# JiuTongBro/vqnerf_release

Measured on AMD Instinct MI355X. Metric: rays/sec (render) 800x800, 64+64 samples/ray, NeuS SDF 8x256 + colour 4x256, higher is better.
Workload: dtype f32; 1 GPU; BASELINE configs[1], nerf/hotdog-shaped NeuS render: one whole 800x800 pin-hole view per rank per step (camera at distance 4, fov 0.6911), n_samples=64, n_importance=64, up_sample_steps=4, sdf 8x256; parallelism=views x1 (no data-path collective)

## Files before the change

vqnerf_release_amd/csrc/mlp_prims.h:

```cpp
#pragma once
#include "common.h"

namespace eng {

enum Act : int { ACT_NONE = 0, ACT_RELU = 1, ACT_SOFTPLUS100 = 2, ACT_SIGMOID = 3 };

__device__ __forceinline__ float fast_exp(float x) { return __builtin_amdgcn_exp2f(x * 1.4426950408889634f); }
__device__ __forceinline__ float fast_log(float x) { return __builtin_amdgcn_logf(x) * 0.6931471805599453f; }
__device__ __forceinline__ float fast_rcp(float x) { return __builtin_amdgcn_rcpf(x); }

template <int ACT>
__device__ __forceinline__ float act_fwd(float x) {
  if (ACT == ACT_RELU) return fmaxf(x, 0.f);
  if (ACT == ACT_SOFTPLUS100) {
    const float t = 100.f * x;
    return t > 20.f ? x : 0.01f * fast_log(1.f + fast_exp(t));
  }
  if (ACT == ACT_SIGMOID) return fast_rcp(1.f + fast_exp(-x));
  return x;
}

template <int ACT>
__device__ __forceinline__ float act_bwd_from_out(float h) {
  if (ACT == ACT_RELU) return h > 0.f ? 1.f : 0.f;
// ... 391 lines not shown
  const f32x4* b = bpack + ot * 8;
  const bool hi = lane >= 32;
#pragma unroll
  for (int rq = 0; rq < 4; ++rq) {
    const f32x4 v0 = b[rq], v1 = b[4 + rq];
    acc[4 * rq + 0] = hi ? v1[0] : v0[0]; acc[4 * rq + 1] = hi ? v1[1] : v0[1];
    acc[4 * rq + 2] = hi ? v1[2] : v0[2]; acc[4 * rq + 3] = hi ? v1[3] : v0[3];
  }
}

__device__ __forceinline__ void init_zero(f32x16& acc) {
#pragma unroll
  for (int i = 0; i < 16; ++i) acc[i] = 0.f;
}

__device__ __forceinline__ void init_rows(const f32x4* __restrict__ rows , int lane, f32x16& acc) {
#pragma unroll
  for (int rq = 0; rq < 4; ++rq) {
    f32x4 v = rows[rq * 64 + lane];
    acc[4 * rq + 0] = v[0]; acc[4 * rq + 1] = v[1]; acc[4 * rq + 2] = v[2]; acc[4 * rq + 3] = v[3];
  }
}

__device__ __forceinline__ float posenc_feat(int f, float x0, float x1, float x2) {
  if (f < 3) return f == 0 ? x0 : (f == 1 ? x1 : x2);
  const int g = f - 3, k = g / 6, m = g - 6 * k, c = m >= 3 ? m - 3 : m;
  const float xc = c == 0 ? x0 : (c == 1 ? x1 : x2);
  const float arg = xc * (float)(1 << k);
  return m < 3 ? sinf(arg) : cosf(arg);
}
__device__ __forceinline__ float posenc_jac(int f, float x0, float x1, float x2, int* comp) {
  if (f < 3) { *comp = f; return 1.f; }
  const int g = f - 3, k = g / 6, m = g - 6 * k, c = m >= 3 ? m - 3 : m;
  const float xc = c == 0 ? x0 : (c == 1 ? x1 : x2);
  const float fr = (float)(1 << k), arg = xc * fr;
  *comp = c;
  return m < 3 ? fr * cosf(arg) : -fr * sinf(arg);
}

__device__ __forceinline__ int row_feat(int r, int h, int j) { return 32 * (r >> 2) + 2 * (4 * (r & 3) + j) + h; }
__device__ __forceinline__ float lds_feat(const f32x4* __restrict__ lds, const int row0, const int f, const int pp) {
  const int t = f >> 5, fi = f & 31, hh = fi & 1, rr = fi >> 1;
  return reinterpret_cast<const float*>(lds)[(((row0 + t * 4 + (rr >> 2)) * 64) + pp + 32 * hh) * 4 + (rr & 3)];
}

template <int NOUT, int NW = 4>
// ... 36 lines not shown
```

vqnerf_release_amd/csrc/neus_launch.h:

```cpp
#pragma once
#include "neus_phases.h"
#include "launch.h"
#include <stdio.h>


static int neus_sdf_args(const char* fn, const int32_t* sdf_desc, const float* wbuf_sdf, const float* rays_o, const float* rays_d,
                         const float* z, const float* pts, const int64_t P, const int S, const float* out_sdf,
                         int (*check_desc)(const SdfDesc&), const char* desc_msg, SdfDesc* sd) {
  VQN_CHECK_ARG_IN(fn, sdf_desc && wbuf_sdf && out_sdf, "sdf_desc, wbuf_sdf, out_sdf must be non-null");
  VQN_CHECK_ARG_IN(fn, P >= 0, "P >= 0");
  if (P == 0) return VQN_OK;
  VQN_CHECK_ARG_IN(fn, pts != nullptr || (rays_o && rays_d && z && S > 0), "either pts or (rays_o, rays_d, z, S) required");
  memcpy(sd, sdf_desc, sizeof(SdfDesc));
  VQN_CHECK_SHAPE_IN(fn, check_desc(*sd) == 0, desc_msg);
  return VQN_OK;
}

static int neus_fine_args(const char* fn, const int32_t* sdf_desc, const float* wbuf_sdf, const int32_t* col_desc, const float* wbuf_col,
                          const float* rays_o, const float* rays_d, const float* z, const float* pts, const float* dirs, const int64_t P,
                          const int S, const void* scratch, const float* out_sdf, const float* out_grad, const float* out_rgb,
                          int (*check_desc)(const SdfDesc&), const char* desc_msg, bool (*extras_rows_ok)(const ColDesc&),
                          SdfDesc* sd, ColDesc* cd) {
  VQN_CHECK_ARG_IN(fn, sdf_desc && wbuf_sdf && col_desc && wbuf_col, "descriptors and weight packs must be non-null");
  VQN_CHECK_ARG_IN(fn, out_sdf && out_grad && scratch, "out_sdf, out_grad and scratch must be non-null");
// ... 8 lines not shown
    VQN_CHECK_ARG_IN(fn, out_rgb != nullptr, "out_rgb must be non-null when a colour net is given");
    VQN_CHECK_SHAPE_IN(fn, sd->layers[sd->n_lin - 1].n_out_tiles >= 1, "SDF network has no feature outputs (d_out == 1)");
    VQN_CHECK_SHAPE_IN(fn, cd->n_lin >= 2 && cd->n_lin <= VQN_MAX_COL_LAYERS && cd->d_out == 3, "colour net: 2..8 layers, d_out == 3");
    VQN_CHECK_SHAPE_IN(fn, cd->extra_feats >= 3 && cd->extra_feats <= 64 && extras_rows_ok(*cd), "colour net extras");
    for (int l = 0; l < cd->n_lin - 1; ++l)
      VQN_CHECK_SHAPE_IN(fn, cd->layers[l].n_out_tiles >= 1 && cd->layers[l].n_out_tiles <= sd->max_tiles, "colour layer wider than max_tiles");
  }
  return VQN_OK;
}

static eng::TrainOut neus_train_out(float* const* tensors, const int nL, const int nC, const int e_tiles, const int outf_tiles, const int extr_tiles) {
  eng::TrainOut to;
  memset(&to, 0, sizeof(to));
  to.E = tensors[0]; to.OUTF = tensors[1]; to.EXTR = tensors[2];
  for (int l = 1; l <= nL; ++l) to.U[l] = tensors[3 + (l - 1)];
  for (int l = 0; l < nL; ++l) to.GH[l] = tensors[3 + nL + l];
  for (int l = 1; l <= nC; ++l) to.C[l] = tensors[3 + 2 * nL + (l - 1)];
  to.e_tiles = e_tiles; to.outf_tiles = outf_tiles; to.extr_tiles = extr_tiles;
  return to;
}

static int64_t neus_stash_bytes(const SdfDesc& sd) { return (int64_t)(sd.n_lin - 1) * 4 * sd.max_tiles * 1024; }

static long pair_grid(const long n_tiles, const int images, const int64_t per_img, const int64_t scratch_bytes) {
  return vqn_grid_in_scratch(vqn_grid((n_tiles + images - 1) / images, images == 1 ? 2 : 1), images * per_img, scratch_bytes);
}

constexpr int TB_MAX_L = 12;

struct TrainBwdDesc {
  int nL, nC, skip, emb_rows, emb_feats, e_tiles, max_tiles, feat_tiles;
  int outf_tiles, squeeze, offBtop, offWrow, offCBfeat, offCBnrm;
  float scale, inv_scale;
  int ts[TB_MAX_L];
  int tc[TB_MAX_L];
  int offT[TB_MAX_L];
  int offB[TB_MAX_L];
  int offCB[TB_MAX_L];
};
constexpr int TB_DESC_INTS = 16 + 5 * TB_MAX_L;
static_assert(sizeof(TrainBwdDesc) == TB_DESC_INTS * 4, "descriptor layout");

struct TrainBwdPtrs {
  const float* X; const float* G_RGB; const float* RGB; const float* G_N; const float* G_SDF;
  const float* U[TB_MAX_L];
  const float* GH[TB_MAX_L];
  const float* C[TB_MAX_L];
  float* DC[TB_MAX_L];
// ... 29 lines not shown
  VQN_CHECK_ARG_IN(fn, desc && w0 && w1 && pts && g_rgb && scratch && saved && outs, "null pointer");
  VQN_CHECK_ARG_IN(fn, P >= 1, "P >= 1");
  VQN_CHECK_SHAPE_IN(fn, train_bwd_load_desc(desc, engine_rules, bd) == 0, desc_msg);
  const int nL = bd->nL, nC = bd->nC;
  VQN_CHECK_ARG_IN(fn, n_saved == 2 * nL + nC, "saved: [U_1..U_nL, GH_0..GH_{nL-1}, C_1..C_nC]");
  VQN_CHECK_ARG_IN(fn, n_outs == (nC + 1) + 2 + 2 * nL, "outs: [DC_0..DC_nC, GOUTF, ED, UD_1..UD_nL, AB_0..AB_{nL-1}]");
  VQN_CHECK_ARG_IN(fn, (rgb != nullptr) == (bd->squeeze != 0), "rgb: the forward's colours when the colour net ends in a sigmoid, else NULL");
  for (int i = 0; i < n_saved; ++i) VQN_CHECK_ARG_IN(fn, saved[i] != nullptr, "null saved tensor");
  for (int i = 0; i < n_outs; ++i) VQN_CHECK_ARG_IN(fn, outs[i] != nullptr, "null output tensor");
  const int64_t per_img = train_bwd_stash_bytes(*bd);
  char scratch_msg[96];
  snprintf(scratch_msg, sizeof(scratch_msg), "scratch too small (see %s_scratch_bytes)", fn);
  VQN_CHECK_ARG_IN(fn, scratch_bytes >= 2 * per_img, scratch_msg);
  memset(tp, 0, sizeof(*tp));
  tp->X = pts; tp->G_RGB = g_rgb; tp->RGB = rgb; tp->G_N = g_n; tp->G_SDF = g_sdf;
  for (int l = 1; l <= nL; ++l) tp->U[l] = saved[l - 1];
  for (int l = 0; l < nL; ++l) tp->GH[l] = saved[nL + l];
  for (int l = 1; l <= nC; ++l) tp->C[l] = saved[2 * nL + l - 1];
  for (int l = 0; l <= nC; ++l) tp->DC[l] = outs[l];
  tp->GOUTF = outs[nC + 1];
  tp->ED = outs[nC + 2];
  for (int l = 1; l <= nL; ++l) tp->UD[l] = outs[nC + 3 + l - 1];
  for (int l = 0; l < nL; ++l) tp->AB[l] = outs[nC + 3 + nL + l];
  *grid = pair_grid((P + 31) / 32, 2, per_img, scratch_bytes);
  return VQN_OK;
}
```

vqnerf_release_amd/csrc/neus_mlp.hip:

```cpp
#include "neus_launch.h"
#include <stdlib.h>

using namespace eng;

#ifdef VQN_STAMPS
__device__ unsigned long long g_stamps[8];
#define VQN_STAMP_DECL unsigned long long st_[6] = {0, 0, 0, 0, 0, 0}; unsigned long long st_prev = __builtin_amdgcn_s_memtime(); const unsigned long long st_begin = st_prev;
#define VQN_STAMP(i) { const unsigned long long st_now = __builtin_amdgcn_s_memtime(); st_[i] += st_now - st_prev; st_prev = st_now; }
#define VQN_STAMP_FLUSH if (threadIdx.x == 0) { st_[5] = __builtin_amdgcn_s_memtime() - st_begin; for (int i_ = 0; i_ < 6; ++i_) atomicAdd(&g_stamps[i_], st_[i_]); atomicAdd(&g_stamps[6], 1ull); }
extern "C" int vqn_debug_read_stamps(unsigned long long* out, int reset) {
  if (hipMemcpyFromSymbol(out, HIP_SYMBOL(g_stamps), sizeof(unsigned long long) * 8) != hipSuccess) return -3;
  if (reset) { unsigned long long z[8] = {0, 0, 0, 0, 0, 0, 0, 0}; if (hipMemcpyToSymbol(HIP_SYMBOL(g_stamps), z, sizeof(z)) != hipSuccess) return -3; }
  return 0;
}
#else
#define VQN_STAMP_DECL
#define VQN_STAMP(i)
#define VQN_STAMP_FLUSH
#endif

#ifdef VQN_STAMPS
__device__ unsigned long long g_stamps2[16];
#define FS_DECL unsigned long long fs_[16] = {0, 0, 0, 0, 0, 0, 0, 0, 0, 0, 0, 0, 0, 0, 0, 0}; unsigned long long fs_prev = __builtin_amdgcn_s_memtime(); const unsigned long long fs_begin = fs_prev;
#define FS(i) { const unsigned long long fs_now = __builtin_amdgcn_s_memtime(); fs_[i] += fs_now - fs_prev; fs_prev = fs_now; }
// ... 610 lines not shown
      if (wave < L.n_out_tiles) {
#pragma unroll
        for (int im = 0; im < NIMG; ++im) {
#pragma unroll
          for (int rq = 0; rq < 4; ++rq) lds[(size_t)im * IS + (X0 + wave * 4 + rq) * 64 + lane] = acc_quad(acc[im], rq);
        }
      }
      __syncthreads();
    }
    const int hid_rows = 4 * sd.layers[n_lin - 2].n_out_tiles;

    for (int u = wave; u < 4 * NIMG; u += 8)
      rowdot<1>(lds + (size_t)(u >> 2) * IS, X0, hid_rows, wsdf + sd.last_w_off, sm->part[u >> 2], u & 3, lane);
    __syncthreads();
    if (tid < 32 * NIMG) {
      const int im = tid >> 5, t = tid & 31;
      const long pt = ((NIMG * grp + im) << 5) + t;
      if (pt < P) out_sdf[pt] = sdf_raw(sm->part[im], t, sd.last_b_off, sd.last_bias, wsdf) / sd.scale;
    }
    __syncthreads();
  }
}

int check_sdf_desc(const SdfDesc& d) {
  if (d.n_lin < 2 || d.n_lin > VQN_MAX_SDF_LAYERS) return 1;
  if (d.max_tiles < 1 || d.max_tiles > 16) return 2;
  if (d.emb_feats < 3 || d.emb_feats > 64 || d.emb_rows < 1 || d.emb_rows > 8) return 3;
  if (d.skip >= d.n_lin - 1 || d.skip == 0) return 4;
  for (int l = 0; l < d.n_lin; ++l)
    if (d.layers[l].n_out_tiles < 0 || d.layers[l].n_out_tiles > d.max_tiles) return 5;
  if (!(d.scale > 0.f)) return 6;
  return 0;
}

template <int NIMG>
size_t lds_bytes(int MT) { return (size_t)NIMG * (E_ROWS + 8 * MT) * 1024 + sizeof(Smalls<NIMG>); }

bool use_two_images(int MT) {
  static const bool forced32 = getenv("VQN_NEUS_TILE32") != nullptr;
  return !forced32 && MT >= 5 && lds_bytes<2>(MT) <= 160 * 1024;
}

template <int NIMG>
size_t lds_bytes_sdf(const SdfDesc& sd) { return (size_t)NIMG * (sd.emb_rows + 4 * sd.max_tiles) * 1024 + sizeof(SmallsSdf<NIMG>); }

constexpr int SDF_IMAGES_DEFAULT = 4;
int sdf_images(const SdfDesc& sd) {
  static const int cap = [] {
    const char* e = getenv("VQN_NEUS_SDF_IMAGES");
    const int v = e != nullptr ? atoi(e) : SDF_IMAGES_DEFAULT;
    return v >= 2 && v <= 4 ? v : SDF_IMAGES_DEFAULT;
  }();
  if (!use_two_images(sd.max_tiles)) return 1;
  if (sd.max_tiles <= 8) {
    if (cap >= 4 && lds_bytes_sdf<4>(sd) <= 160 * 1024) return 4;
    if (cap >= 3 && lds_bytes_sdf<3>(sd) <= 160 * 1024) return 3;
  }
  return 2;
}

template <int NIMG>
int launch_sdf_images(const char* fn, const SdfDesc& sd, const f32x4* ws, const float* rays_o, const float* rays_d, const float* z,
                      const float* pts, const int64_t P, const int S, float* out_sdf, void* stream) {
  return vqn_launch(fn, neus_pointsN_kernel<NIMG>, pair_grid((P + 31) / 32, NIMG, 0, 0), 512, lds_bytes_sdf<NIMG>(sd), stream, sd, ws,
                    rays_o, rays_d, z, pts, (long)P, S, out_sdf);
}

bool extras_rows_ok(const ColDesc& cd) { return cd.extra_rows >= 1 && cd.extra_rows <= 8; }

}

extern "C" int vqn_neus_sdf_points(const int32_t* sdf_desc, const float* wbuf_sdf, const float* rays_o,
                                   const float* rays_d, const float* z, const float* pts, int64_t P, int S,
                                   float* out_sdf, void* stream) {
  SdfDesc sd;
  const int rc = neus_sdf_args(__func__, sdf_desc, wbuf_sdf, rays_o, rays_d, z, pts, P, S, out_sdf, check_sdf_desc,
                               "invalid SDF network descriptor", &sd);
  if (rc != VQN_OK || P == 0) return rc;
  ColDesc cd;
  memset(&cd, 0, sizeof(cd));
  const long n_tiles = (P + 31) / 32;
  const f32x4* ws = reinterpret_cast<const f32x4*>(wbuf_sdf);
  const int images = sdf_images(sd);
  if (images == 4) return launch_sdf_images<4>(__func__, sd, ws, rays_o, rays_d, z, pts, P, S, out_sdf, stream);
  if (images == 3) return launch_sdf_images<3>(__func__, sd, ws, rays_o, rays_d, z, pts, P, S, out_sdf, stream);
  if (images == 2)
    return vqn_launch(__func__, neus_points2_kernel<false>, pair_grid(n_tiles, 2, 0, 0), 512, lds_bytes<2>(sd.max_tiles), stream, sd, cd, ws,
                      nullptr, rays_o, rays_d, z, pts, nullptr, (long)P, S, nullptr, out_sdf, nullptr, nullptr, TrainOut{});
  const size_t lds = lds_bytes<1>(sd.max_tiles);
  VQN_CHECK_SHAPE(lds <= 160 * 1024, "network too wide for LDS");
  return vqn_launch(__func__, neus_points_kernel<false>, pair_grid(n_tiles, 1, 0, 0), 256, lds, stream, sd, cd, ws, nullptr, rays_o, rays_d,
                    z, pts, nullptr, (long)P, S, nullptr, out_sdf, nullptr, nullptr);
}

extern "C" int vqn_neus_train_fwd(const int32_t* sdf_desc, const float* wbuf_sdf, const int32_t* col_desc, const float* wbuf_col,
                                  const float* pts, const float* dirs, int64_t P, void* scratch, int64_t scratch_bytes,
                                  float* const* tensors, int n_tensors, int e_tiles, int outf_tiles, int extr_tiles, float* out_sdf,
                                  float* out_n, float* out_rgb, void* stream) {
  VQN_CHECK_ARG(sdf_desc && wbuf_sdf && col_desc && wbuf_col && pts && dirs && scratch && tensors && out_sdf && out_n && out_rgb, "null pointer");
  VQN_CHECK_ARG(P >= 1, "P >= 1");
  SdfDesc sd;
  ColDesc cd;
  memcpy(&sd, sdf_desc, sizeof(SdfDesc));
  memcpy(&cd, col_desc, sizeof(ColDesc));
  VQN_CHECK_SHAPE(check_sdf_desc(sd) == 0, "invalid SDF network descriptor");
  VQN_CHECK_SHAPE(cd.n_lin >= 2 && cd.n_lin <= VQN_MAX_COL_LAYERS && cd.d_out == 3 && sd.layers[sd.n_lin - 1].n_out_tiles >= 1, "colour net");
  VQN_CHECK_SHAPE(use_two_images(sd.max_tiles), "the training forward kernel is the two-image form only");
  const int nL = sd.n_lin - 1, nC = cd.n_lin - 1;
  VQN_CHECK_ARG(n_tensors == 3 + 2 * nL + nC, "tensors: [E, OUTF, EXTR, U_1..U_nL, GH_0..GH_{nL-1}, C_1..C_nC]");
  VQN_CHECK_SHAPE(e_tiles * 4 >= sd.emb_rows && e_tiles <= 2 && extr_tiles * 4 >= cd.extra_rows && extr_tiles <= 2 &&
                  outf_tiles >= sd.layers[sd.n_lin - 1].n_out_tiles, "tile counts");
  for (int i = 0; i < n_tensors; ++i) VQN_CHECK_ARG(tensors[i] != nullptr, "null tensor pointer");
  const long grid = pair_grid((P + 31) / 32, 2, neus_stash_bytes(sd), scratch_bytes);
  VQN_CHECK_ARG(grid >= 1, "scratch too small (see vqn_neus_fine_scratch_bytes)");
  return vqn_launch(__func__, neus_points2_kernel<true, true>, grid, 512, lds_bytes<2>(sd.max_tiles), stream, sd, cd,
                    reinterpret_cast<const f32x4*>(wbuf_sdf), reinterpret_cast<const f32x4*>(wbuf_col), nullptr, nullptr, nullptr, pts, dirs,
                    (long)P, 1, reinterpret_cast<f32x4*>(scratch), out_sdf, out_n, out_rgb,
                    neus_train_out(tensors, nL, nC, e_tiles, outf_tiles, extr_tiles));
}

extern "C" int64_t vqn_neus_fine_scratch_bytes(const int32_t* sdf_desc) {
  if (!sdf_desc) return -1;
  SdfDesc sd;
  memcpy(&sd, sdf_desc, sizeof(SdfDesc));
  const int emb_rows = sd.emb_rows;
  if (emb_rows >= 1 && emb_rows <= 12) sd.emb_rows = 1;
  if (check_sdf_desc(sd) != 0) return -2;
#ifdef VQN_DIAG_STASH_ROT
  return (int64_t)VQN_DIAG_STASH_ROT * vqn_num_cus() * 2 * neus_stash_bytes(sd);
#else
  return (int64_t)vqn_num_cus() * 2 * neus_stash_bytes(sd);
#endif
}

extern "C" int vqn_neus_fine_points(const int32_t* sdf_desc, const float* wbuf_sdf, const int32_t* col_desc,
                                    const float* wbuf_col, const float* rays_o, const float* rays_d, const float* z,
                                    const float* pts, const float* dirs, int64_t P, int S, void* scratch,
                                    int64_t scratch_bytes, float* out_sdf, float* out_grad, float* out_rgb,
                                    void* stream) {
  SdfDesc sd;
  ColDesc cd;
  const int rc = neus_fine_args(__func__, sdf_desc, wbuf_sdf, col_desc, wbuf_col, rays_o, rays_d, z, pts, dirs, P, S, scratch, out_sdf,
                                out_grad, out_rgb, check_sdf_desc, "invalid SDF network descriptor", extras_rows_ok, &sd, &cd);
  if (rc != VQN_OK || P == 0) return rc;
  if (cd.n_lin != 0)
    VQN_CHECK_ARG((cd.reserved1 > 0 && cd.reserved2 > cd.reserved1 && cd.reserved3 > cd.reserved2) ||
                  (cd.reserved1 == 0 && cd.reserved2 == 0 && cd.reserved3 == 0), "col_desc: fold offsets (reserved1..3) inconsistent");
  const long n_tiles = (P + 31) / 32;
  const int64_t per_img = neus_stash_bytes(sd);
  const f32x4* ws = reinterpret_cast<const f32x4*>(wbuf_sdf);
  const f32x4* wc = reinterpret_cast<const f32x4*>(wbuf_col);
  if (use_two_images(sd.max_tiles)) {
    const bool fold = cd.n_lin != 0 && cd.reserved1 > 0;
#ifdef VQN_DIAG_STASH_ROT
    const long grid = pair_grid(n_tiles, 2, 0, 0);
    VQN_CHECK_ARG((int64_t)VQN_DIAG_STASH_ROT * grid * 2 * per_img <= scratch_bytes, "diag build: scratch must hold ROT regions per workgroup");
#else
    const long grid = pair_grid(n_tiles, 2, per_img, scratch_bytes);
#endif
    VQN_CHECK_ARG(grid >= 1, "scratch too small (see vqn_neus_fine_scratch_bytes)");
    return vqn_launch(__func__, fold ? neus_points2_kernel<true, false, true> : neus_points2_kernel<true>, grid, 512, lds_bytes<2>(sd.max_tiles),
                      stream, sd, cd, ws, wc, rays_o, rays_d, z, pts, dirs, (long)P, S, reinterpret_cast<f32x4*>(scratch), out_sdf, out_grad,
                      out_rgb, TrainOut{});
  }
  const size_t lds = lds_bytes<1>(sd.max_tiles);
  VQN_CHECK_SHAPE(lds <= 160 * 1024, "network too wide for LDS");
  const long grid = pair_grid(n_tiles, 1, per_img, scratch_bytes);
  VQN_CHECK_ARG(grid >= 1, "scratch too small (see vqn_neus_fine_scratch_bytes)");
  return vqn_launch(__func__, neus_points_kernel<true>, grid, 256, lds, stream, sd, cd, ws, wc, rays_o, rays_d, z, pts, dirs, (long)P, S,
                    reinterpret_cast<f32x4*>(scratch), out_sdf, out_grad, out_rgb);
}
```

vqnerf_release_amd/csrc/neus_mlp_f16s.hip:

```cpp
#include "mlp_prims_f16s.h"
#include "neus_launch.h"
#include <stdlib.h>

using namespace eng;

#define st_stream(p, ...) (*(p) = (__VA_ARGS__))
#define ld_stream(p) (*(p))

#ifdef VQN_STAMPS
__device__ unsigned long long g_stamps16[16];
#define FS_DECL unsigned long long st_[16] = {0, 0, 0, 0, 0, 0, 0, 0, 0, 0, 0, 0, 0, 0, 0, 0}; unsigned long long st_prev = __builtin_amdgcn_s_memtime(); const unsigned long long st_begin = st_prev;
#define FS(i) { const unsigned long long st_now = __builtin_amdgcn_s_memtime(); st_[i] += st_now - st_prev; st_prev = st_now; }
#define FS_FLUSH if (threadIdx.x == 0) { st_[14] = __builtin_amdgcn_s_memtime() - st_begin; for (int i_ = 0; i_ < 15; ++i_) atomicAdd(&g_stamps16[i_], st_[i_]); atomicAdd(&g_stamps16[15], 1ull); }
extern "C" int vqn_debug_read_stamps16(unsigned long long* out, int reset) {
  if (hipMemcpyFromSymbol(out, HIP_SYMBOL(g_stamps16), sizeof(unsigned long long) * 16) != hipSuccess) return -3;
  if (reset) { unsigned long long z[16] = {0}; if (hipMemcpyToSymbol(HIP_SYMBOL(g_stamps16), z, sizeof(z)) != hipSuccess) return -3; }
  return 0;
}
#else
#define FS_DECL
#define FS(i)
#define FS_FLUSH
#endif

// ... 345 lines not shown

bool use_two_images(int MT) {
  static const bool forced32 = getenv("VQN_F16S_TILE32") != nullptr;
  return !forced32 && lds_bytes<2>(MT) <= 160 * 1024;
}

bool extras_rows_ok(const ColDesc& cd) { return cd.extra_rows >= 2 && cd.extra_rows <= 8 && !(cd.extra_rows & 1); }

constexpr const char* DESC_MSG = "invalid SDF network descriptor (split-precision packs have even row counts)";

}

extern "C" int vqn_neus_sdf_points_f16s(const int32_t* sdf_desc, const float* wbuf_sdf, const float* rays_o,
                                        const float* rays_d, const float* z, const float* pts, int64_t P, int S,
                                        float* out_sdf, void* stream) {
  SdfDesc sd;
  const int rc = neus_sdf_args(__func__, sdf_desc, wbuf_sdf, rays_o, rays_d, z, pts, P, S, out_sdf, check_sdf_desc, DESC_MSG, &sd);
  if (rc != VQN_OK || P == 0) return rc;
  ColDesc cd;
  memset(&cd, 0, sizeof(cd));
  const long n_tiles = (P + 31) / 32;
  const f32x4* ws = reinterpret_cast<const f32x4*>(wbuf_sdf);
  if (use_two_images(sd.max_tiles))
    return vqn_launch(__func__, neus_points_f16s_kernel<false, 2>, pair_grid(n_tiles, 2, 0, 0), 512, lds_bytes<2>(sd.max_tiles), stream, sd, cd,
                      ws, nullptr, rays_o, rays_d, z, pts, nullptr, (long)P, S, nullptr, out_sdf, nullptr, nullptr);
  const size_t lds = lds_bytes<1>(sd.max_tiles);
  VQN_CHECK_SHAPE(lds <= 160 * 1024, "network too wide for LDS");
  return vqn_launch(__func__, neus_points_f16s_kernel<false, 1>, pair_grid(n_tiles, 1, 0, 0), 256, lds, stream, sd, cd, ws, nullptr, rays_o,
                    rays_d, z, pts, nullptr, (long)P, S, nullptr, out_sdf, nullptr, nullptr);
}

extern "C" int vqn_neus_fine_points_f16s(const int32_t* sdf_desc, const float* wbuf_sdf, const int32_t* col_desc,
                                         const float* wbuf_col, const float* rays_o, const float* rays_d, const float* z,
                                         const float* pts, const float* dirs, int64_t P, int S, void* scratch,
                                         int64_t scratch_bytes, float* out_sdf, float* out_grad, float* out_rgb,
                                         void* stream) {
  SdfDesc sd;
  ColDesc cd;
  const int rc = neus_fine_args(__func__, sdf_desc, wbuf_sdf, col_desc, wbuf_col, rays_o, rays_d, z, pts, dirs, P, S, scratch, out_sdf,
                                out_grad, out_rgb, check_sdf_desc, DESC_MSG, extras_rows_ok, &sd, &cd);
  if (rc != VQN_OK || P == 0) return rc;
  const long n_tiles = (P + 31) / 32;
  const f32x4* ws = reinterpret_cast<const f32x4*>(wbuf_sdf);
  const f32x4* wc = reinterpret_cast<const f32x4*>(wbuf_col);
  if (use_two_images(sd.max_tiles)) {
    const long grid = pair_grid(n_tiles, 2, neus_stash_bytes(sd), scratch_bytes);
    VQN_CHECK_ARG(grid >= 1, "scratch too small (see vqn_neus_fine_scratch_bytes)");
    return vqn_launch(__func__, neus_points_f16s_kernel<true, 2>, grid, 512, lds_bytes<2>(sd.max_tiles), stream, sd, cd, ws, wc, rays_o, rays_d,
                      z, pts, dirs, (long)P, S, reinterpret_cast<f32x4*>(scratch), out_sdf, out_grad, out_rgb);
  }
  const size_t lds = lds_bytes<1>(sd.max_tiles);
  VQN_CHECK_SHAPE(lds <= 160 * 1024, "network too wide for LDS");
  const long grid = pair_grid(n_tiles, 1, neus_stash_bytes(sd), scratch_bytes);
  VQN_CHECK_ARG(grid >= 1, "scratch too small (see vqn_neus_fine_scratch_bytes)");
  return vqn_launch(__func__, neus_points_f16s_kernel<true, 1>, grid, 256, lds, stream, sd, cd, ws, wc, rays_o, rays_d, z, pts, dirs, (long)P,
                    S, reinterpret_cast<f32x4*>(scratch), out_sdf, out_grad, out_rgb);
}
```

vqnerf_release_amd/csrc/neus_mlp_x3.hip:

```cpp
#include "mlp_prims_x3.h"
#include "neus_launch.h"
#include <stdlib.h>

using namespace eng;

#define VQN_X3_HV_EARLY 1

namespace {

constexpr int E0 = 0;
constexpr int E_ROWS = 12;
constexpr int X0 = E_ROWS;
constexpr int MAX_CALLS = 40;
constexpr int RING = 2;
constexpr int NW = 8;

struct SmallsTab : Smalls<2> {
  int tab[MAX_CALLS * 4];
  int n_calls;
};

template <bool FINE, int NACC, bool TRAIN = false>
__global__ __launch_bounds__(512, 1) void neus_points_x3_kernel(
    const SdfDesc sd, const ColDesc cd, const f32x4* __restrict__ wsdf, const f32x4* __restrict__ wcol,
// ... 362 lines not shown

int x3_nacc() {
  static const int n = [] { const char* e = getenv("VQN_X3_NACC"); return (e && e[0] == '1') ? 1 : 2; }();
  return n;
}

bool extras_rows_ok(const ColDesc& cd) { return cd.extra_rows == x3_rows(cd.extra_feats); }

constexpr const char* DESC_MSG = "invalid SDF network descriptor for the x3 engine (x3 packs: 3 rows per 16 features; layers of at most 256 outputs)";

}

extern "C" int vqn_neus_sdf_points_x3(const int32_t* sdf_desc, const float* wbuf_sdf, const float* rays_o,
                                      const float* rays_d, const float* z, const float* pts, int64_t P, int S,
                                      float* out_sdf, void* stream) {
  SdfDesc sd;
  const int rc = neus_sdf_args(__func__, sdf_desc, wbuf_sdf, rays_o, rays_d, z, pts, P, S, out_sdf, check_sdf_desc_x3, DESC_MSG, &sd);
  if (rc != VQN_OK || P == 0) return rc;
  ColDesc cd;
  memset(&cd, 0, sizeof(cd));
  const size_t lds2 = lds_bytes_x3(sd.max_tiles);
  VQN_CHECK_SHAPE(lds2 <= 160 * 1024, "network too wide for LDS");
  return vqn_launch(__func__, x3_nacc() == 2 ? neus_points_x3_kernel<false, 2> : neus_points_x3_kernel<false, 1>,
                    pair_grid((P + 31) / 32, 2, 0, 0), 512, lds2, stream, sd, cd, reinterpret_cast<const f32x4*>(wbuf_sdf), nullptr, rays_o,
                    rays_d, z, pts, nullptr, (long)P, S, nullptr, out_sdf, nullptr, nullptr, TrainOut{});
}

extern "C" int vqn_neus_fine_points_x3(const int32_t* sdf_desc, const float* wbuf_sdf, const int32_t* col_desc,
                                       const float* wbuf_col, const float* rays_o, const float* rays_d, const float* z,
                                       const float* pts, const float* dirs, int64_t P, int S, void* scratch,
                                       int64_t scratch_bytes, float* out_sdf, float* out_grad, float* out_rgb,
                                       void* stream) {
  SdfDesc sd;
  ColDesc cd;
  const int rc = neus_fine_args(__func__, sdf_desc, wbuf_sdf, col_desc, wbuf_col, rays_o, rays_d, z, pts, dirs, P, S, scratch, out_sdf,
                                out_grad, out_rgb, check_sdf_desc_x3, DESC_MSG, extras_rows_ok, &sd, &cd);
  if (rc != VQN_OK || P == 0) return rc;
  const size_t lds2 = lds_bytes_x3(sd.max_tiles);
  VQN_CHECK_SHAPE(lds2 <= 160 * 1024, "network too wide for LDS");
  const long grid = pair_grid((P + 31) / 32, 2, neus_stash_bytes(sd), scratch_bytes);
  VQN_CHECK_ARG(grid >= 1, "scratch too small (see vqn_neus_fine_scratch_bytes)");
  return vqn_launch(__func__, x3_nacc() == 2 ? neus_points_x3_kernel<true, 2> : neus_points_x3_kernel<true, 1>, grid, 512, lds2, stream, sd,
                    cd, reinterpret_cast<const f32x4*>(wbuf_sdf), reinterpret_cast<const f32x4*>(wbuf_col), rays_o, rays_d, z, pts, dirs,
                    (long)P, S, reinterpret_cast<f32x4*>(scratch), out_sdf, out_grad, out_rgb, TrainOut{});
}

extern "C" int vqn_neus_train_fwd_x3(const int32_t* sdf_desc, const float* wbuf_sdf, const int32_t* col_desc, const float* wbuf_col,
                                     const float* pts, const float* dirs, int64_t P, void* scratch, int64_t scratch_bytes,
                                     float* const* tensors, int n_tensors, int e_tiles, int outf_tiles, int extr_tiles, float* out_sdf,
                                     float* out_n, float* out_rgb, void* stream) {
  VQN_CHECK_ARG(sdf_desc && wbuf_sdf && col_desc && wbuf_col && pts && dirs && scratch && tensors && out_sdf && out_n && out_rgb, "null pointer");
  VQN_CHECK_ARG(P >= 1, "P >= 1");
  SdfDesc sd;
  ColDesc cd;
  memcpy(&sd, sdf_desc, sizeof(SdfDesc));
  memcpy(&cd, col_desc, sizeof(ColDesc));
  VQN_CHECK_SHAPE(check_sdf_desc_x3(sd) == 0, "invalid SDF network descriptor for the x3 engine");
  VQN_CHECK_SHAPE(cd.n_lin >= 2 && cd.n_lin <= VQN_MAX_COL_LAYERS && cd.d_out == 3 && sd.layers[sd.n_lin - 1].n_out_tiles >= 1, "colour net");
  VQN_CHECK_SHAPE(cd.extra_feats >= 3 && cd.extra_feats <= 64 && extras_rows_ok(cd), "colour net extras");
  for (int l = 0; l < cd.n_lin - 1; ++l)
    VQN_CHECK_SHAPE(cd.layers[l].n_out_tiles >= 1 && cd.layers[l].n_out_tiles <= sd.max_tiles, "colour layer wider than max_tiles");
  const int nL = sd.n_lin - 1, nC = cd.n_lin - 1;
  VQN_CHECK_ARG(n_tensors == 3 + 2 * nL + nC, "tensors: [E, OUTF, EXTR, U_1..U_nL, GH_0..GH_{nL-1}, C_1..C_nC]");
  VQN_CHECK_SHAPE(2 * e_tiles * 3 >= sd.emb_rows && e_tiles <= 2 && 2 * extr_tiles * 3 >= cd.extra_rows && extr_tiles <= 2 &&
                  outf_tiles >= sd.layers[sd.n_lin - 1].n_out_tiles, "tile counts");
  for (int i = 0; i < n_tensors; ++i) VQN_CHECK_ARG(tensors[i] != nullptr, "null tensor pointer");
  const size_t lds2 = lds_bytes_x3(sd.max_tiles);
  VQN_CHECK_SHAPE(lds2 <= 160 * 1024, "network too wide for LDS");
  const long grid = pair_grid((P + 31) / 32, 2, neus_stash_bytes(sd), scratch_bytes);
  VQN_CHECK_ARG(grid >= 1, "scratch too small (see vqn_neus_fine_scratch_bytes)");
  return vqn_launch(__func__, x3_nacc() == 2 ? neus_points_x3_kernel<true, 2, true> : neus_points_x3_kernel<true, 1, true>, grid, 512, lds2,
                    stream, sd, cd, reinterpret_cast<const f32x4*>(wbuf_sdf), reinterpret_cast<const f32x4*>(wbuf_col), nullptr, nullptr,
                    nullptr, pts, dirs, (long)P, 1, reinterpret_cast<f32x4*>(scratch), out_sdf, out_n, out_rgb,
                    neus_train_out(tensors, nL, nC, e_tiles, outf_tiles, extr_tiles));
}
```

Measured before the change: 283,300 rays/s.

## Add 256-thread two-image fine-point kernel with in-place LDS layers, two WGs per CU

Adds a new fine-pass NeuS kernel that processes two 32-point tiles with 256 threads (4 waves) instead of 512. Each layer's output overwrites its input region in LDS, which halves the per-image activation footprint and lets two workgroups share a CU. It becomes the default when the network fits (max_tiles ≤ 8 and two copies fit in LDS), and the scratch sizing doubles to hold stash regions for two workgroups per CU. The cost is an extra barrier per layer for the in-place writeback and fewer waves sharing each weight load.

After: 286,700 rays/s, median of 6. 1.2% higher.

```diff
diff --git a/vqnerf_release_amd/csrc/mlp_prims.h b/vqnerf_release_amd/csrc/mlp_prims.h
--- a/vqnerf_release_amd/csrc/mlp_prims.h
+++ b/vqnerf_release_amd/csrc/mlp_prims.h
@@ -437,6 +437,32 @@
   }
 }
 
+template <class Init, class Epi>
+__device__ __forceinline__ void gemm_tiles2_in_place(f32x4* __restrict__ lds, const int img_stride, const KSegs ks,
+                                                     const f32x4* __restrict__ w, const int n_out_tiles, const int wave, const int lane,
+                                                     const int dst_row0, Init init, Epi epi) {
+  f32x4 held0[2][4], held1[2][4], nopre[4];
+  gemm_tiles2<4>(lds, img_stride, ks, w, n_out_tiles, wave, lane, nopre, false, nullptr, init,
+                 [&](int ot, int im, int rq, const f32x16& acc) {
+                   f32x4 v = {acc[4 * rq], acc[4 * rq + 1], acc[4 * rq + 2], acc[4 * rq + 3]};
+                   epi(ot, im, rq, v);
+                   if (ot == wave) held0[im][rq] = v; else held1[im][rq] = v;
+                 });
+  __syncthreads();
+#pragma unroll
+  for (int im = 0; im < 2; ++im) {
+    if (wave < n_out_tiles) {
+#pragma unroll
+      for (int rq = 0; rq < 4; ++rq) lds[im * img_stride + (dst_row0 + wave * 4 + rq) * 64 + lane] = held0[im][rq];
+    }
+    if (wave + 4 < n_out_tiles) {
+#pragma unroll
+      for (int rq = 0; rq < 4; ++rq) lds[im * img_stride + (dst_row0 + (wave + 4) * 4 + rq) * 64 + lane] = held1[im][rq];
+    }
+  }
+  __syncthreads();
+}
+
 __device__ __forceinline__ float posenc_feat(int f, float x0, float x1, float x2) {
   if (f < 3) return f == 0 ? x0 : (f == 1 ? x1 : x2);
   const int g = f - 3, k = g / 6, m = g - 6 * k, c = m >= 3 ? m - 3 : m;
diff --git a/vqnerf_release_amd/csrc/neus_launch.h b/vqnerf_release_amd/csrc/neus_launch.h
--- a/vqnerf_release_amd/csrc/neus_launch.h
+++ b/vqnerf_release_amd/csrc/neus_launch.h
@@ -54,8 +54,8 @@
 
 static int64_t neus_stash_bytes(const SdfDesc& sd) { return (int64_t)(sd.n_lin - 1) * 4 * sd.max_tiles * 1024; }
 
-static long pair_grid(const long n_tiles, const int images, const int64_t per_img, const int64_t scratch_bytes) {
-  return vqn_grid_in_scratch(vqn_grid((n_tiles + images - 1) / images, images == 1 ? 2 : 1), images * per_img, scratch_bytes);
+static long pair_grid(const long n_tiles, const int images, const int per_cu, const int64_t per_img, const int64_t scratch_bytes) {
+  return vqn_grid_in_scratch(vqn_grid((n_tiles + images - 1) / images, per_cu), images * per_img, scratch_bytes);
 }
 
 constexpr int TB_MAX_L = 12;
@@ -131,6 +131,6 @@
   tp->ED = outs[nC + 2];
   for (int l = 1; l <= nL; ++l) tp->UD[l] = outs[nC + 3 + l - 1];
   for (int l = 0; l < nL; ++l) tp->AB[l] = outs[nC + 3 + nL + l];
-  *grid = pair_grid((P + 31) / 32, 2, per_img, scratch_bytes);
+  *grid = pair_grid((P + 31) / 32, 2, 1, per_img, scratch_bytes);
   return VQN_OK;
 }
diff --git a/vqnerf_release_amd/csrc/neus_mlp.hip b/vqnerf_release_amd/csrc/neus_mlp.hip
--- a/vqnerf_release_amd/csrc/neus_mlp.hip
+++ b/vqnerf_release_amd/csrc/neus_mlp.hip
@@ -656,6 +656,234 @@
   }
 }
 
+struct SmallsW {
+  float pts[2][96], dirs[2][96], part[2][384], grad[2][96];
+};
+
+__device__ __forceinline__ void wte_in_place(f32x4* __restrict__ lds, const int IS, const int k_row0, const int ng,
+                                             const f32x4* __restrict__ w, const int emb_tiles, const int KS, const int e_row0,
+                                             const int e_rows, const bool accumulate, const int wave, const int lane) {
+  const int gk = (ng + KS - 1) / KS;
+  for (int u = wave; u < 2 * emb_tiles; u += 4) {
+    const int t = u % emb_tiles;
+    f32x4* li = lds + (size_t)(u / emb_tiles) * IS;
+    const f32x4* __restrict__ wp = w + (size_t)t * ng * 64 + lane;
+    f32x16 sum;
+    for (int k = 0; k < KS; ++k) {
+      f32x16 acc;
+      init_zero(acc);
+      const int g0 = k * gk, g1 = min(ng, g0 + gk);
+      for (int g = g0; g < g1; g += 8) {
+        f32x4 a[8], b[8];
+#pragma unroll
+        for (int i = 0; i < 8; ++i) {
+          const int gg = min(g + i, ng - 1);
+          a[i] = wp[gg * 64]; b[i] = li[(k_row0 + gg) * 64 + lane];
+        }
+#pragma unroll
+        for (int i = 0; i < 8; ++i)
+          if (g + i < g1) {
+#pragma unroll
+            for (int j = 0; j < 4; ++j) acc = __builtin_amdgcn_mfma_f32_32x32x2f32(a[i][j], b[i][j], acc, 0, 0, 0);
+          }
+      }
+      if (k == 0) sum = acc; else sum += acc;
+    }
+#pragma unroll
+    for (int rq = 0; rq < 4; ++rq)
+      if (t * 4 + rq < e_rows) {
+        f32x4 v = acc_quad(sum, rq);
+        if (accumulate) v += li[(e_row0 + t * 4 + rq) * 64 + lane];
+        li[(e_row0 + t * 4 + rq) * 64 + lane] = v;
+      }
+  }
+}
+
+template <bool FOLD>
+__global__ __launch_bounds__(256, 2) void neus_points2w_kernel(
+    const SdfDesc sd, const ColDesc cd, const f32x4* __restrict__ wsdf, const f32x4* __restrict__ wcol,
+    const float* __restrict__ rays_o, const float* __restrict__ rays_d, const float* __restrict__ zv,
+    const float* __restrict__ pts_direct, const float* __restrict__ dirs_direct, const long P, const int S,
+    f32x4* __restrict__ scratch, float* __restrict__ out_sdf, float* __restrict__ out_grad,
+    float* __restrict__ out_rgb) {
+  extern __shared__ __attribute__((aligned(16))) f32x4 lds[];
+  const int MT = sd.max_tiles;
+  const int X0 = max(sd.emb_rows, cd.extra_rows);
+  const int IS = (X0 + 4 * MT) * 64;
+  SmallsW* sm = reinterpret_cast<SmallsW*>(lds + (size_t)2 * IS);
+  const int tid = threadIdx.x, lane = tid & 63, h = lane >> 5, p = lane & 31;
+  const int wave = __builtin_amdgcn_readfirstlane(tid >> 6);
+  const int n_lin = sd.n_lin;
+  const int emb_tiles = (sd.emb_feats + 31) >> 5;
+  const int ks_wte = min(8, MT) / emb_tiles;
+  const long n_tiles = (P + 31) >> 5, n_pairs = (n_tiles + 1) >> 1;
+  const size_t per_img = (size_t)(n_lin - 1) * 4 * MT * 64;
+  f32x4* save0 = scratch + (size_t)blockIdx.x * 2 * per_img;
+  const int feat_slot = (n_lin - 2) * 4 * MT;
+  f32x4 nopre[4];
+
+  for (long pair = blockIdx.x; pair < n_pairs; pair += gridDim.x) {
+    if (tid < 64) {
+      const int im = tid >> 5, t = tid & 31;
+      load_point<true>(((2 * pair + im) << 5) + t, P, S, rays_o, rays_d, zv, pts_direct, dirs_direct, sm->pts[im] + t * 3, sm->dirs[im] + t * 3);
+    }
+    __syncthreads();
+    for (int u = wave; u < 2 * sd.emb_rows; u += 4) {
+      const int im = u / sd.emb_rows, r = u - im * sd.emb_rows;
+      const float xs = sm->pts[im][p * 3 + 0] * sd.scale, ys = sm->pts[im][p * 3 + 1] * sd.scale, zs = sm->pts[im][p * 3 + 2] * sd.scale;
+      f32x4 v;
+#pragma unroll
+      for (int j = 0; j < 4; ++j) v[j] = emb_feat(row_feat(r, h, j), sd.emb_feats, xs, ys, zs);
+      lds[(size_t)im * IS + (E0 + r) * 64 + lane] = v;
+    }
+    __syncthreads();
+
+    for (int l = 0; l < n_lin - 1; ++l) {
+      const LayerDesc L = sd.layers[l];
+      const KSegs ks = (l == 0) ? KSegs{E0, sd.emb_rows, 0, 0}
+                                : KSegs{X0, 4 * sd.layers[l - 1].n_out_tiles, E0, (l == sd.skip) ? sd.emb_rows : 0};
+      const bool do_save = l < n_lin - 2;
+      const f32x4* bp = wsdf + L.b_off;
+      gemm_tiles2_in_place(lds, IS, ks, wsdf + L.w_off, L.n_out_tiles, wave, lane, X0,
+                           [&](int ot, int, f32x16& acc) { init_bias(bp, ot, lane, acc); },
+                           [&](int ot, int im, int rq, f32x4& v) {
+#pragma unroll
+                             for (int j = 0; j < 4; ++j) v[j] = act_fwd<ACT_SOFTPLUS100>(v[j]);
+                             if (do_save) st_stream(save0 + (size_t)im * per_img + (size_t)l * 4 * MT * 64 + (ot * 4 + rq) * 64 + lane, v);
+                           });
+    }
+    const int hid_rows = 4 * sd.layers[n_lin - 2].n_out_tiles;
+
+    for (int im = 0; im < 2; ++im) rowdot<1>(lds + (size_t)im * IS, X0, hid_rows, wsdf + sd.last_w_off, sm->part[im], wave, lane);
+    if (sd.layers[n_lin - 1].n_out_tiles > 0) {
+      const LayerDesc L = sd.layers[n_lin - 1];
+      const f32x4* bp = FOLD ? wcol + cd.reserved2 : wsdf + L.b_off;
+      gemm_tiles2<4>(lds, IS, KSegs{X0, hid_rows, 0, 0}, FOLD ? wcol + cd.reserved1 : wsdf + L.w_off,
+                     FOLD ? cd.layers[0].n_out_tiles : L.n_out_tiles, wave, lane, nopre, false, nullptr,
+                     [&](int ot, int, f32x16& acc) { init_bias(bp, ot, lane, acc); },
+                     [&](int ot, int im, int rq, const f32x16& acc) {
+                       st_stream(save0 + (size_t)im * per_img + (size_t)feat_slot * 64 + (ot * 4 + rq) * 64 + lane, acc_quad(acc, rq));
+                     });
+    }
+    __syncthreads();
+    if (tid < 64) {
+      const int im = tid >> 5, t = tid & 31;
+      const long pt = ((2 * pair + im) << 5) + t;
+      if (pt < P) out_sdf[pt] = sdf_raw(sm->part[im], t, sd.last_b_off, sd.last_bias, wsdf) / sd.scale;
+    }
+    for (int im = 0; im < 2; ++im) {
+      f32x4* li = lds + (size_t)im * IS;
+      for (int r0 = wave; r0 < hid_rows; r0 += 32) {
+        f32x4 v[8], wv[8];
+#pragma unroll
+        for (int c = 0; c < 8; ++c) {
+          const int r = min(r0 + 4 * c, hid_rows - 1);
+          v[c] = li[(X0 + r) * 64 + lane];
+          wv[c] = wsdf[sd.last_w_off + r * 2 + h];
+        }
+#pragma unroll
+        for (int c = 0; c < 8; ++c)
+          if (r0 + 4 * c < hid_rows) {
+#pragma unroll
+            for (int j = 0; j < 4; ++j) v[c][j] = wv[c][j] * act_bwd_from_out<ACT_SOFTPLUS100>(v[c][j]);
+            li[(X0 + r0 + 4 * c) * 64 + lane] = v[c];
+          }
+      }
+    }
+    __syncthreads();
+    for (int l = n_lin - 2; l >= 1; --l) {
+      const LayerDesc L = sd.layers[l];
+      if (l == sd.skip)
+        wte_in_place(lds, IS, X0, 4 * L.n_out_tiles, wsdf + L.wTE_off, emb_tiles, ks_wte, E0, sd.emb_rows, false, wave, lane);
+      f32x4 hv[2][4];
+      gemm_tiles2_in_place(lds, IS, KSegs{X0, 4 * L.n_out_tiles, 0, 0}, wsdf + L.wT_off, sd.layers[l - 1].n_out_tiles, wave, lane, X0,
+                           [&](int ot, int im, f32x16& acc) {
+                             const f32x4* sv = save0 + (size_t)im * per_img + (size_t)(l - 1) * 4 * MT * 64;
+#pragma unroll
+                             for (int rq = 0; rq < 4; ++rq) hv[im][rq] = ld_stream(sv + (ot * 4 + rq) * 64 + lane);
+                             init_zero(acc);
+                           },
+                           [&](int, int im, int rq, f32x4& v) {
+#pragma unroll
+                             for (int j = 0; j < 4; ++j) v[j] *= act_bwd_from_out<ACT_SOFTPLUS100>(hv[im][rq][j]);
+                           });
+    }
+    wte_in_place(lds, IS, X0, 4 * sd.layers[0].n_out_tiles, wsdf + sd.layers[0].wTE_off, emb_tiles, ks_wte, E0, sd.emb_rows, sd.skip >= 1,
+                 wave, lane);
+    __syncthreads();
+    if (tid < 192) {
+      const int im = tid / 96, r = tid - 96 * im, pp = r & 31, c = r >> 5;
+      const f32x4* li = lds + (size_t)im * IS;
+      const float g = embed_chain([&](int f) { return lds_feat(li, E0, f, pp); }, c, sd.multires, sm->pts[im] + pp * 3, sd.scale);
+      sm->grad[im][pp * 3 + c] = g;
+      const long pt = ((2 * pair + im) << 5) + pp;
+      if (pt < P) out_grad[pt * 3 + c] = g;
+    }
+    __syncthreads();
+    if (cd.n_lin == 0) continue;
+
+    const int feat_rows = 4 * sd.layers[n_lin - 1].n_out_tiles;
+    for (int im = 0; im < 2; ++im) {
+      f32x4* li = lds + (size_t)im * IS;
+      const float px = sm->pts[im][p * 3 + 0], py = sm->pts[im][p * 3 + 1], pz = sm->pts[im][p * 3 + 2];
+      const float dx = sm->dirs[im][p * 3 + 0], dy = sm->dirs[im][p * 3 + 1], dz = sm->dirs[im][p * 3 + 2];
+      for (int r = wave; r < cd.extra_rows; r += 4) {
+        f32x4 v;
+#pragma unroll
+        for (int j = 0; j < 4; ++j)
+          v[j] = col_extra_feat(row_feat(r, h, j), px, py, pz, dx, dy, dz, sm->grad[im] + p * 3, cd.n_view_feats, cd.extra_feats);
+        li[(E0 + r) * 64 + lane] = v;
+      }
+      const f32x4* sv = save0 + (size_t)im * per_img + (size_t)feat_slot * 64;
+      for (int r0 = wave; r0 < (FOLD ? 0 : feat_rows); r0 += 32) {
+        f32x4 v[8];
+#pragma unroll
+        for (int c = 0; c < 8; ++c) v[c] = ld_stream(sv + min(r0 + 4 * c, feat_rows - 1) * 64 + lane);
+#pragma unroll
+        for (int c = 0; c < 8; ++c)
+          if (r0 + 4 * c < feat_rows) li[(X0 + r0 + 4 * c) * 64 + lane] = v[c];
+      }
+    }
+    __syncthreads();
+    int in_rows = feat_rows;
+    auto relu = [&](int, int, int, f32x4& v) {
+#pragma unroll
+      for (int j = 0; j < 4; ++j) v[j] = act_fwd<ACT_RELU>(v[j]);
+    };
+    if (FOLD) {
+      const LayerDesc L = cd.layers[0];
+      gemm_tiles2_in_place(lds, IS, KSegs{E0, cd.extra_rows, 0, 0}, wcol + cd.reserved3, L.n_out_tiles, wave, lane, X0,
+                           [&](int ot, int im, f32x16& acc) {
+                             const f32x4* pp = save0 + (size_t)im * per_img + (size_t)feat_slot * 64 + ot * 256 + lane;
+#pragma unroll
+                             for (int rq = 0; rq < 4; ++rq) {
+                               const f32x4 v = ld_stream(pp + rq * 64);
+                               acc[4 * rq + 0] = v[0]; acc[4 * rq + 1] = v[1]; acc[4 * rq + 2] = v[2]; acc[4 * rq + 3] = v[3];
+                             }
+                           },
+                           relu);
+      in_rows = 4 * L.n_out_tiles;
+    }
+    for (int l = FOLD ? 1 : 0; l < cd.n_lin - 1; ++l) {
+      const LayerDesc L = cd.layers[l];
+      const f32x4* bp = wcol + L.b_off;
+      gemm_tiles2_in_place(lds, IS, KSegs{X0, in_rows, E0, l == 0 ? cd.extra_rows : 0}, wcol + L.w_off, L.n_out_tiles, wave, lane, X0,
+                           [&](int ot, int, f32x16& acc) { init_bias(bp, ot, lane, acc); }, relu);
+      in_rows = 4 * L.n_out_tiles;
+    }
+    for (int im = 0; im < 2; ++im) rowdot<3>(lds + (size_t)im * IS, X0, in_rows, wcol + cd.last_w_off, sm->part[im], wave, lane);
+    __syncthreads();
+    if (tid < 192) {
+      const int im = tid / 96, r = tid - 96 * im, pp = r & 31, o = r >> 5;
+      const float v = rgb_out(sm->part[im], pp, o, cd.last_b_off, cd.last_bias[o], cd.squeeze_out, wcol);
+      const long pt = ((2 * pair + im) << 5) + pp;
+      if (pt < P) out_rgb[pt * 3 + o] = v;
+    }
+    __syncthreads();
+  }
+}
+
+
 int check_sdf_desc(const SdfDesc& d) {
   if (d.n_lin < 2 || d.n_lin > VQN_MAX_SDF_LAYERS) return 1;
   if (d.max_tiles < 1 || d.max_tiles > 16) return 2;
@@ -696,8 +924,20 @@
 template <int NIMG>
 int launch_sdf_images(const char* fn, const SdfDesc& sd, const f32x4* ws, const float* rays_o, const float* rays_d, const float* z,
                       const float* pts, const int64_t P, const int S, float* out_sdf, void* stream) {
-  return vqn_launch(fn, neus_pointsN_kernel<NIMG>, pair_grid((P + 31) / 32, NIMG, 0, 0), 512, lds_bytes_sdf<NIMG>(sd), stream, sd, ws,
+  return vqn_launch(fn, neus_pointsN_kernel<NIMG>, pair_grid((P + 31) / 32, NIMG, 1, 0, 0), 512, lds_bytes_sdf<NIMG>(sd), stream, sd, ws,
                     rays_o, rays_d, z, pts, (long)P, S, out_sdf);
+}
+
+size_t lds_bytes_wg(const SdfDesc& sd, const int extra_rows) {
+  return (size_t)2 * ((sd.emb_rows > extra_rows ? sd.emb_rows : extra_rows) + 4 * sd.max_tiles) * 1024 + sizeof(SmallsW);
+}
+
+bool use_wg_form(const SdfDesc& sd, const int extra_rows) {
+  static const bool images = [] {
+    const char* e = getenv("VQN_NEUS_FORM");
+    return e != nullptr && strcmp(e, "images") == 0;
+  }();
+  return !images && use_two_images(sd.max_tiles) && sd.max_tiles <= 8 && 2 * lds_bytes_wg(sd, extra_rows) <= 160 * 1024;
 }
 
 bool extras_rows_ok(const ColDesc& cd) { return cd.extra_rows >= 1 && cd.extra_rows <= 8; }
@@ -719,11 +959,11 @@
   if (images == 4) return launch_sdf_images<4>(__func__, sd, ws, rays_o, rays_d, z, pts, P, S, out_sdf, stream);
   if (images == 3) return launch_sdf_images<3>(__func__, sd, ws, rays_o, rays_d, z, pts, P, S, out_sdf, stream);
   if (images == 2)
-    return vqn_launch(__func__, neus_points2_kernel<false>, pair_grid(n_tiles, 2, 0, 0), 512, lds_bytes<2>(sd.max_tiles), stream, sd, cd, ws,
+    return vqn_launch(__func__, neus_points2_kernel<false>, pair_grid(n_tiles, 2, 1, 0, 0), 512, lds_bytes<2>(sd.max_tiles), stream, sd, cd, ws,
                       nullptr, rays_o, rays_d, z, pts, nullptr, (long)P, S, nullptr, out_sdf, nullptr, nullptr, TrainOut{});
   const size_t lds = lds_bytes<1>(sd.max_tiles);
   VQN_CHECK_SHAPE(lds <= 160 * 1024, "network too wide for LDS");
-  return vqn_launch(__func__, neus_points_kernel<false>, pair_grid(n_tiles, 1, 0, 0), 256, lds, stream, sd, cd, ws, nullptr, rays_o, rays_d,
+  return vqn_launch(__func__, neus_points_kernel<false>, pair_grid(n_tiles, 1, 2, 0, 0), 256, lds, stream, sd, cd, ws, nullptr, rays_o, rays_d,
                     z, pts, nullptr, (long)P, S, nullptr, out_sdf, nullptr, nullptr);
 }
 
@@ -745,7 +985,7 @@
   VQN_CHECK_SHAPE(e_tiles * 4 >= sd.emb_rows && e_tiles <= 2 && extr_tiles * 4 >= cd.extra_rows && extr_tiles <= 2 &&
                   outf_tiles >= sd.layers[sd.n_lin - 1].n_out_tiles, "tile counts");
   for (int i = 0; i < n_tensors; ++i) VQN_CHECK_ARG(tensors[i] != nullptr, "null tensor pointer");
-  const long grid = pair_grid((P + 31) / 32, 2, neus_stash_bytes(sd), scratch_bytes);
+  const long grid = pair_grid((P + 31) / 32, 2, 1, neus_stash_bytes(sd), scratch_bytes);
   VQN_CHECK_ARG(grid >= 1, "scratch too small (see vqn_neus_fine_scratch_bytes)");
   return vqn_launch(__func__, neus_points2_kernel<true, true>, grid, 512, lds_bytes<2>(sd.max_tiles), stream, sd, cd,
                     reinterpret_cast<const f32x4*>(wbuf_sdf), reinterpret_cast<const f32x4*>(wbuf_col), nullptr, nullptr, nullptr, pts, dirs,
@@ -763,7 +1003,7 @@
 #ifdef VQN_DIAG_STASH_ROT
   return (int64_t)VQN_DIAG_STASH_ROT * vqn_num_cus() * 2 * neus_stash_bytes(sd);
 #else
-  return (int64_t)vqn_num_cus() * 2 * neus_stash_bytes(sd);
+  return (int64_t)vqn_num_cus() * (use_wg_form(sd, 0) ? 4 : 2) * neus_stash_bytes(sd);
 #endif
 }
 
@@ -784,13 +1024,21 @@
   const int64_t per_img = neus_stash_bytes(sd);
   const f32x4* ws = reinterpret_cast<const f32x4*>(wbuf_sdf);
   const f32x4* wc = reinterpret_cast<const f32x4*>(wbuf_col);
+  if (use_wg_form(sd, cd.extra_rows)) {
+    const bool fold = cd.n_lin != 0 && cd.reserved1 > 0;
+    const long grid = pair_grid(n_tiles, 2, 2, per_img, scratch_bytes);
+    VQN_CHECK_ARG(grid >= 1, "scratch too small (see vqn_neus_fine_scratch_bytes)");
+    return vqn_launch(__func__, fold ? neus_points2w_kernel<true> : neus_points2w_kernel<false>, grid, 256,
+                      lds_bytes_wg(sd, cd.extra_rows), stream, sd, cd, ws, wc, rays_o, rays_d, z, pts, dirs, (long)P, S,
+                      reinterpret_cast<f32x4*>(scratch), out_sdf, out_grad, out_rgb);
+  }
   if (use_two_images(sd.max_tiles)) {
     const bool fold = cd.n_lin != 0 && cd.reserved1 > 0;
 #ifdef VQN_DIAG_STASH_ROT
-    const long grid = pair_grid(n_tiles, 2, 0, 0);
+    const long grid = pair_grid(n_tiles, 2, 1, 0, 0);
     VQN_CHECK_ARG((int64_t)VQN_DIAG_STASH_ROT * grid * 2 * per_img <= scratch_bytes, "diag build: scratch must hold ROT regions per workgroup");
 #else
-    const long grid = pair_grid(n_tiles, 2, per_img, scratch_bytes);
+    const long grid = pair_grid(n_tiles, 2, 1, per_img, scratch_bytes);
 #endif
     VQN_CHECK_ARG(grid >= 1, "scratch too small (see vqn_neus_fine_scratch_bytes)");
     return vqn_launch(__func__, fold ? neus_points2_kernel<true, false, true> : neus_points2_kernel<true>, grid, 512, lds_bytes<2>(sd.max_tiles),
@@ -799,7 +1047,7 @@
   }
   const size_t lds = lds_bytes<1>(sd.max_tiles);
   VQN_CHECK_SHAPE(lds <= 160 * 1024, "network too wide for LDS");
-  const long grid = pair_grid(n_tiles, 1, per_img, scratch_bytes);
+  const long grid = pair_grid(n_tiles, 1, 2, per_img, scratch_bytes);
   VQN_CHECK_ARG(grid >= 1, "scratch too small (see vqn_neus_fine_scratch_bytes)");
   return vqn_launch(__func__, neus_points_kernel<true>, grid, 256, lds, stream, sd, cd, ws, wc, rays_o, rays_d, z, pts, dirs, (long)P, S,
                     reinterpret_cast<f32x4*>(scratch), out_sdf, out_grad, out_rgb);
diff --git a/vqnerf_release_amd/csrc/neus_mlp_f16s.hip b/vqnerf_release_amd/csrc/neus_mlp_f16s.hip
--- a/vqnerf_release_amd/csrc/neus_mlp_f16s.hip
+++ b/vqnerf_release_amd/csrc/neus_mlp_f16s.hip
@@ -391,11 +391,11 @@
   const long n_tiles = (P + 31) / 32;
   const f32x4* ws = reinterpret_cast<const f32x4*>(wbuf_sdf);
   if (use_two_images(sd.max_tiles))
-    return vqn_launch(__func__, neus_points_f16s_kernel<false, 2>, pair_grid(n_tiles, 2, 0, 0), 512, lds_bytes<2>(sd.max_tiles), stream, sd, cd,
+    return vqn_launch(__func__, neus_points_f16s_kernel<false, 2>, pair_grid(n_tiles, 2, 1, 0, 0), 512, lds_bytes<2>(sd.max_tiles), stream, sd, cd,
                       ws, nullptr, rays_o, rays_d, z, pts, nullptr, (long)P, S, nullptr, out_sdf, nullptr, nullptr);
   const size_t lds = lds_bytes<1>(sd.max_tiles);
   VQN_CHECK_SHAPE(lds <= 160 * 1024, "network too wide for LDS");
-  return vqn_launch(__func__, neus_points_f16s_kernel<false, 1>, pair_grid(n_tiles, 1, 0, 0), 256, lds, stream, sd, cd, ws, nullptr, rays_o,
+  return vqn_launch(__func__, neus_points_f16s_kernel<false, 1>, pair_grid(n_tiles, 1, 2, 0, 0), 256, lds, stream, sd, cd, ws, nullptr, rays_o,
                     rays_d, z, pts, nullptr, (long)P, S, nullptr, out_sdf, nullptr, nullptr);
 }
 
@@ -413,14 +413,14 @@
   const f32x4* ws = reinterpret_cast<const f32x4*>(wbuf_sdf);
   const f32x4* wc = reinterpret_cast<const f32x4*>(wbuf_col);
   if (use_two_images(sd.max_tiles)) {
-    const long grid = pair_grid(n_tiles, 2, neus_stash_bytes(sd), scratch_bytes);
+    const long grid = pair_grid(n_tiles, 2, 1, neus_stash_bytes(sd), scratch_bytes);
     VQN_CHECK_ARG(grid >= 1, "scratch too small (see vqn_neus_fine_scratch_bytes)");
     return vqn_launch(__func__, neus_points_f16s_kernel<true, 2>, grid, 512, lds_bytes<2>(sd.max_tiles), stream, sd, cd, ws, wc, rays_o, rays_d,
                       z, pts, dirs, (long)P, S, reinterpret_cast<f32x4*>(scratch), out_sdf, out_grad, out_rgb);
   }
   const size_t lds = lds_bytes<1>(sd.max_tiles);
   VQN_CHECK_SHAPE(lds <= 160 * 1024, "network too wide for LDS");
-  const long grid = pair_grid(n_tiles, 1, neus_stash_bytes(sd), scratch_bytes);
+  const long grid = pair_grid(n_tiles, 1, 2, neus_stash_bytes(sd), scratch_bytes);
   VQN_CHECK_ARG(grid >= 1, "scratch too small (see vqn_neus_fine_scratch_bytes)");
   return vqn_launch(__func__, neus_points_f16s_kernel<true, 1>, grid, 256, lds, stream, sd, cd, ws, wc, rays_o, rays_d, z, pts, dirs, (long)P,
                     S, reinterpret_cast<f32x4*>(scratch), out_sdf, out_grad, out_rgb);
diff --git a/vqnerf_release_amd/csrc/neus_mlp_x3.hip b/vqnerf_release_amd/csrc/neus_mlp_x3.hip
--- a/vqnerf_release_amd/csrc/neus_mlp_x3.hip
+++ b/vqnerf_release_amd/csrc/neus_mlp_x3.hip
@@ -408,7 +408,7 @@
   const size_t lds2 = lds_bytes_x3(sd.max_tiles);
   VQN_CHECK_SHAPE(lds2 <= 160 * 1024, "network too wide for LDS");
   return vqn_launch(__func__, x3_nacc() == 2 ? neus_points_x3_kernel<false, 2> : neus_points_x3_kernel<false, 1>,
-                    pair_grid((P + 31) / 32, 2, 0, 0), 512, lds2, stream, sd, cd, reinterpret_cast<const f32x4*>(wbuf_sdf), nullptr, rays_o,
+                    pair_grid((P + 31) / 32, 2, 1, 0, 0), 512, lds2, stream, sd, cd, reinterpret_cast<const f32x4*>(wbuf_sdf), nullptr, rays_o,
                     rays_d, z, pts, nullptr, (long)P, S, nullptr, out_sdf, nullptr, nullptr, TrainOut{});
 }
 
@@ -424,7 +424,7 @@
   if (rc != VQN_OK || P == 0) return rc;
   const size_t lds2 = lds_bytes_x3(sd.max_tiles);
   VQN_CHECK_SHAPE(lds2 <= 160 * 1024, "network too wide for LDS");
-  const long grid = pair_grid((P + 31) / 32, 2, neus_stash_bytes(sd), scratch_bytes);
+  const long grid = pair_grid((P + 31) / 32, 2, 1, neus_stash_bytes(sd), scratch_bytes);
   VQN_CHECK_ARG(grid >= 1, "scratch too small (see vqn_neus_fine_scratch_bytes)");
   return vqn_launch(__func__, x3_nacc() == 2 ? neus_points_x3_kernel<true, 2> : neus_points_x3_kernel<true, 1>, grid, 512, lds2, stream, sd,
                     cd, reinterpret_cast<const f32x4*>(wbuf_sdf), reinterpret_cast<const f32x4*>(wbuf_col), rays_o, rays_d, z, pts, dirs,
@@ -453,7 +453,7 @@
   for (int i = 0; i < n_tensors; ++i) VQN_CHECK_ARG(tensors[i] != nullptr, "null tensor pointer");
   const size_t lds2 = lds_bytes_x3(sd.max_tiles);
   VQN_CHECK_SHAPE(lds2 <= 160 * 1024, "network too wide for LDS");
-  const long grid = pair_grid((P + 31) / 32, 2, neus_stash_bytes(sd), scratch_bytes);
+  const long grid = pair_grid((P + 31) / 32, 2, 1, neus_stash_bytes(sd), scratch_bytes);
   VQN_CHECK_ARG(grid >= 1, "scratch too small (see vqn_neus_fine_scratch_bytes)");
   return vqn_launch(__func__, x3_nacc() == 2 ? neus_points_x3_kernel<true, 2, true> : neus_points_x3_kernel<true, 1, true>, grid, 512, lds2,
                     stream, sd, cd, reinterpret_cast<const f32x4*>(wbuf_sdf), reinterpret_cast<const f32x4*>(wbuf_col), nullptr, nullptr,
```
